# cliangyu/video-diffusion

Hardware: AMD Instinct MI355X
Metric: denoise-steps/sec (higher is better)
Workload: dtype f32

## Files before the change

### include/vd_amd.h

```cpp
#ifndef VD_AMD_H
#define VD_AMD_H
#ifdef __cplusplus
extern "C" {
#endif

typedef struct vd_config {
    int image_size;
    int num_channels;
    int num_res_blocks;
    int num_heads;
    int T;
    int n_attention_ds;
    int attention_ds[8];
    int use_scale_shift_norm;
    int use_spatial_encoding;
    int use_frame_encoding;
    int enforce_position_invariance;
    int use_rpe_net;
    int allow_interactions_between_padding;
    float rp_alpha, rp_beta, rp_gamma;
    int time_embed_mult;
    int cond_emb_type;
    int learn_sigma;
} vd_config;
// ... 71 lines not shown
                     double* mse_out, void* stream);
int vd_op_eps_mse(vd_engine* e, int B, int T, const float* x_start, const float* eps, const long long* t, int clip_denoised,
                  const float* latent_mask, unsigned long long seed, const unsigned long long* item_offset, const float* noise,
                  double* mse_out, void* stream);

int vd_window_begin(vd_engine* e, int B, int T, float* x, const float* obs_src, const float* obs_mask,
                    const float* latent_mask, const float* kinda_marg_mask, const long long* frame_indices,
                    int observed_frames, int sampler, int clip_denoised, float eta, unsigned long long seed,
                    unsigned long long offset, long long t_start, void* stream);
int vd_window_run(vd_engine* e, int n_steps, void* stream);
unsigned long long vd_window_generation(vd_engine* e);
int vd_window_graphs(vd_engine* e);

int vd_set_window_prefix_cache(vd_engine* e, int on);
int vd_window_prefix_frames(vd_engine* e);

int vd_set_window_suffix_skip(vd_engine* e, int on);
int vd_window_suffix_frames(vd_engine* e);

int vd_posterior_update(vd_engine* e, int mode, int B, long long per_sample, const float* x, const float* eps,
                        const long long* t, int clip_denoised, float eta, const float* noise,
                        unsigned long long seed, unsigned long long offset, float* sample, float* pred_xstart,
                        void* stream);

int vd_posterior_from_xstart(vd_engine* e, int mode, int B, long long per_sample, const float* x, const float* xstart_in,
                             const long long* t, int clip_denoised, float eta, const float* noise,
                             unsigned long long seed, unsigned long long offset, float* sample, float* pred_xstart,
                             float* mean, void* stream);

int vd_attn_blocks(vd_engine* e);
// ... 71 lines not shown
int vd_op_gn_bwd(const float* x0, const float* x1, int C0, int C, const float* affA, const float* affB, const float* mr,
                 const float* dy, int act, int nfr, int HW, const float* extra, float* dx0, int acc0, float* dx1, int acc1,
                 void* stream);
int vd_op_gn_temporal_bwd(const float* x, const float* gamma, const float* dy, int B, int T, int HW, int C, int accumulate,
                          float* dx, void* stream);
int vd_op_attn_temporal_bwd(const float* qkv, const float* Rk, const float* Rq, const float* Rv, const float* mask, int B,
                            int T, int HW, int C, int heads, int allow_pad, const float* dout, float* dqkv, void* stream);
int vd_op_attn_spatial_bwd(const float* qkv, int nfr, int L, int C, int heads, const float* dout, float* dqkv, void* stream);
int vd_op_out_conv_bwd(const float* deps, const float* w, int nfr, int H, int W, int C, int Cout, float* da, void* stream);
int vd_op_stem_col2im(const float* dcols, const float* obs, const float* lat, const float* km, int nfr, int H, int W,
                      int cond_mode, float* dx, void* stream);
int vd_op_sinus_embed(const float* t, int n, int dim, const float* freqs, float* out, void* stream);
int vd_op_frame_t(const long long* frame_indices, int B, int T, int center, float* tv, void* stream);
int vd_op_rpe_hidden(const float* te, int te_ld, const float* wbase, const long long* tab, const long long* frame_indices, int B, int T,
                     int C, float* E, int nz, long long zs_e, void* stream);
int vd_op_rpe_table(const float* table, const long long* frame_indices, int B, int T, int C, float alpha, float beta, float gamma,
                    float* R, void* stream);
int vd_op_posenc_add(const float* x, const float* P, const float* femb, int nfr, int HW, int C, float* y, void* stream);
int vd_op_assemble(const float* x, const float* obs_src, const float* obs_mask, const float* latent_mask, const float* kinda_marg_mask,
                   const float* t_model, int obs_t_mode, int B, int T, int H, int W, int Kpad, int cond_mode, const int* frame_list,
                   int n_list, int scalars_only, float* x_cols, float* t_frames, float* amask, void* stream);
int vd_op_move_rows(int scatter, const float* src, const int* list, int n, long long row_floats, float* dst, void* stream);
int vd_op_scatter_stats(const double* src, int split, int C, const int* list, int n, double* dst, void* stream);

typedef struct vd_lpips vd_lpips;
int vd_lpips_create(vd_lpips** out);
void vd_lpips_destroy(vd_lpips* h);
int vd_lpips_load_weight(vd_lpips* h, const char* name, const float* host, long long bytes);
long long vd_lpips_dim(int H, int W);
int vd_lpips_embed(vd_lpips* h, int N, int H, int W, const float* frames, float* out, void* stream);
// ... 28 lines not shown
```

### video-diffusion_amd/_lib.py

```python
import ctypes
import os
import subprocess

_HERE = os.path.dirname(os.path.abspath(__file__))
_CSRC = os.path.join(_HERE, "csrc")
SO_PATH = os.path.join(_HERE, "libvdamd.so")
SOURCES = ["igemm.hip", "conv_wino.hip", "conv_wino_r64.hip", "conv_wino_z128.hip", "gemm_frag.hip", "gemm_split.hip", "split_pack.hip", "norm.hip", "backward.hip", "attn_spatial.hip", "attn_temporal.hip", "attn_temporal_long.hip", "misc.hip", "engine.hip", "lpips.hip", "metrics.hip", "i3d.hip", "conv_cl.hip", "hallway.hip"]
HEADER = os.path.join(os.path.dirname(_HERE), "include", "vd_amd.h")
HEADERS = [os.path.join(_CSRC, "vd_common.h"), os.path.join(_CSRC, "wino_common.h"), os.path.join(_CSRC, "igemm_tile.h"), HEADER]
SOURCE_FLAGS = {"conv_wino_z128.hip": ["-mllvm", "-pragma-unroll-threshold=1000000"]}


def _toolchain():
    hipcc = os.environ.get("HIPCC", "/opt/rocm/bin/hipcc")
    flags = ["--offload-arch=gfx950", "-O3", "-std=c++17", "-fPIC", "-Wno-unused-value"] + \
        os.environ.get("VD_HIPCC_FLAGS", "").split()
    return hipcc, flags


def _sha(*parts):
    import hashlib
    h = hashlib.sha1()
    for p in parts:
        h.update(p if isinstance(p, bytes) else str(p).encode())
# ... 115 lines not shown
    "vd_pos_channels": (_I, [_P]),
    "vd_pos_resolution": (_I, [_P]),
    "vd_set_freqs": (_I, [_P, _P, _I, _P, _I]),
    "vd_set_schedule": (_I, [_P, _I, _P, _P, _F]),
    "vd_workspace_bytes": (_I, [_P, _I, _I, ctypes.POINTER(_L)]),
    "vd_unet_forward": (_I, [_P, _I, _I, _P, _P, _P, _P, _P, _P, _P, _I, _P, _P]),
    "vd_p_sample": (_I, [_P, _I, _I, _P, _P, _P, _P, _P, _P, _P, _I, _I, _P, _U, _U, _P, _P, _P, _P]),
    "vd_ddim_sample": (_I, [_P, _I, _I, _P, _P, _P, _P, _P, _P, _P, _I, _I, _F, _P, _U, _U, _P, _P, _P, _P]),
    "vd_p_mean_variance": (_I, [_P, _I, _I, _P, _P, _P, _P, _P, _P, _P, _I, _I, _P, _P, _P, _P]),
    "vd_vb_terms": (_I, [_P, _I, _I, _P, _P, _P, _P, _P, _I, _P, _P, _P, _P, _P, _P]),
    "vd_prior_bpd": (_I, [_P, _I, _I, _P, _P, _P, _P]),
    "vd_score_windows": (_I, [_P, _I, _I, _P, _P, _P, _P, _P, _P, _I, _U, _P, _P, _I, _P, _P]),
    "vd_op_eps_mse": (_I, [_P, _I, _I, _P, _P, _P, _I, _P, _U, _P, _P, _P, _P]),
    "vd_window_generation": (_U, [_P]),
    "vd_set_window_prefix_cache": (_I, [_P, _I]),
    "vd_window_prefix_frames": (_I, [_P]),
    "vd_set_window_suffix_skip": (_I, [_P, _I]),
    "vd_window_suffix_frames": (_I, [_P]),
    "vd_window_begin": (_I, [_P, _I, _I, _P, _P, _P, _P, _P, _P, _I, _I, _I, _F, _U, _U, _L, _P]),
    "vd_window_run": (_I, [_P, _I, _P]),
    "vd_window_graphs": (_I, [_P]),
    "vd_posterior_update": (_I, [_P, _I, _I, _L, _P, _P, _P, _I, _F, _P, _U, _U, _P, _P, _P]),
    "vd_posterior_from_xstart": (_I, [_P, _I, _I, _L, _P, _P, _P, _I, _F, _P, _U, _U, _P, _P, _P, _P]),
    "vd_attn_blocks": (_I, [_P]),
    "vd_attn_block_info": (_I, [_P, _I, ctypes.POINTER(_I), ctypes.POINTER(_I)]),
    "vd_set_attn_capture": (_I, [_P, _P, _P, _I]),
    "vd_bwd_weights_bytes": (_L, [_P]),
    "vd_set_bwd_weight_storage": (_I, [_P, _P, _L, _I]),
    "vd_load_weight_bwd": (_I, [_P, ctypes.c_char_p, _P, _L]),
    "vd_guided_step": (_I, [_P, _I, _I, _P, _P, _P, _P, _P, _P, _I, _P, _P, _P, _P, _P, _P, _P, _P]),
# ... 30 lines not shown
    "vd_op_affine_apply": (_I, [_P, _P, _P, _I, _I, _I, _P, _P]),
    "vd_op_affine_act": (_I, [_P, _P, _I, _I, _P, _P, _I, _I, _I, _P, _P]),
    "vd_op_gn_temporal": (_I, [_P, _P, _P, _I, _I, _I, _I, _P, _P]),
    "vd_op_attn_spatial": (_I, [_P, _I, _I, _I, _I, _P, _P]),
    "vd_op_attn_temporal": (_I, [_P, _P, _P, _P, _P, _I, _I, _I, _I, _I, _I, _P, _P]),
    "vd_op_out_conv": (_I, [_P, _P, _P, _P, _P, _I, _I, _I, _I, _I, _P, _P]),
    "vd_op_gn_bwd": (_I, [_P, _P, _I, _I, _P, _P, _P, _P, _I, _I, _I, _P, _P, _I, _P, _I, _P]),
    "vd_op_gn_temporal_bwd": (_I, [_P, _P, _P, _I, _I, _I, _I, _I, _P, _P]),
    "vd_op_attn_temporal_bwd": (_I, [_P, _P, _P, _P, _P, _I, _I, _I, _I, _I, _I, _P, _P, _P]),
    "vd_op_attn_spatial_bwd": (_I, [_P, _I, _I, _I, _I, _P, _P, _P]),
    "vd_op_out_conv_bwd": (_I, [_P, _P, _I, _I, _I, _I, _I, _P, _P]),
    "vd_op_stem_col2im": (_I, [_P, _P, _P, _P, _I, _I, _I, _I, _P, _P]),
    "vd_op_sinus_embed": (_I, [_P, _I, _I, _P, _P, _P]),
    "vd_op_frame_t": (_I, [_P, _I, _I, _I, _P, _P]),
    "vd_op_rpe_hidden": (_I, [_P, _I, _P, _P, _P, _I, _I, _I, _P, _I, _L, _P]),
    "vd_op_rpe_table": (_I, [_P, _P, _I, _I, _I, _F, _F, _F, _P, _P]),
    "vd_op_posenc_add": (_I, [_P, _P, _P, _I, _I, _I, _P, _P]),
    "vd_op_assemble": (_I, [_P, _P, _P, _P, _P, _P, _I, _I, _I, _I, _I, _I, _I, _P, _I, _I, _P, _P, _P, _P]),
    "vd_op_move_rows": (_I, [_I, _P, _P, _I, _L, _P, _P]),
    "vd_op_scatter_stats": (_I, [_P, _I, _I, _P, _I, _P, _P]),
    "vd_lpips_create": (_I, [ctypes.POINTER(_P)]),
    "vd_lpips_destroy": (None, [_P]),
    "vd_lpips_load_weight": (_I, [_P, ctypes.c_char_p, _P, _L]),
    "vd_lpips_dim": (_L, [_I, _I]),
    "vd_lpips_embed": (_I, [_P, _I, _I, _I, _P, _P, _P]),
    "vd_fps_select": (_I, [_I, _I, _L, _P, _I, _P, _I, _P, _P, _P]),
    "vd_frame_metrics": (_I, [_I, _I, _I, _I, _P, _P, _I, _D, _P, _P, _P]),
    "vd_pair_sqdist": (_I, [_I, _L, _P, _P, _P, _P]),
    "vd_i3d_create": (_I, [ctypes.POINTER(_P)]),
    "vd_i3d_destroy": (None, [_P]),
# ... 55 lines not shown
```

### video-diffusion_amd/csrc/engine.hip

```cpp
#include <cmath>
#include <cstring>
#include <unordered_map>
#include <vector>

#include "../../include/vd_amd.h"
#include "vd_common.h"

namespace vd {

thread_local std::string g_last_error;
void set_error(const std::string& msg) { g_last_error = msg; }

int launch_frame_t(const int64_t* fidx, int B, int T, int center, float* tv, hipStream_t s);

enum ParamKind { PK_RAW = 0, PK_CONV3, PK_STEM, PK_POSENC, PK_OUTCONV, PK_LINF, PK_CONV3W, PK_CONV3S,
                 PK_CONV3WU };

struct Param {
    std::string name;
    int nd = 0;
    long long shape[4] = {1, 1, 1, 1};
    size_t numel = 0;
    size_t packed = 0;
    size_t off = 0;
// ... 176 lines not shown
    int suf_blk = -2, suf_layer = -1;
    int p_posenc = -1, p_te0w, p_te0b, p_te2w, p_te2b, p_outgw, p_outgb, p_outw, p_outb;
    size_t film_w_off = 0, film_b_off = 0, te_w_off = 0, te_b_off = 0;
    int film_total = 0, te_total = 0;
    size_t packed_total = 0;
    float* wbuf = nullptr;
    bool wbuf_on_host = false;
    int put(void* dst, const void* src, size_t bytes) {
        if (wbuf_on_host) { std::memcpy(dst, src, bytes); return 0; }
        VD_HIP(hipMemcpy(dst, src, bytes, hipMemcpyHostToDevice));
        return 0;
    }
    struct RpeGroup { int C; std::vector<int> blocks; long long* d_hid = nullptr; long long* d_out = nullptr; };
    std::vector<RpeGroup> rpe_groups;
    std::vector<float*> rpe_R;
    int rpe_all(const float* te, const int64_t* fidx, int B, int T, hipStream_t st, Arena& ar);
    int rpe_tables();
    void rpe_group_blocks();
    float* d_freq_time = nullptr; int n_freq_time = 0;
    float* d_freq_frame = nullptr; int n_freq_frame = 0;
    float* d_tab = nullptr; int num_timesteps = 0;
    float* d_tmap = nullptr; float rescale = 1.f;
    char* ws = nullptr; size_t ws_cap = 0;
    bool ws_suf = false;
    int ws_B = 0, ws_T = 0; size_t ws_tail = 0;
    std::unordered_map<long long, size_t> ws_peaks;
    static size_t tm_bytes(int B) { return ((size_t)B * sizeof(float) + 255) & ~(size_t)255; }
    size_t step_tail_bytes(int B, int T) const { return tm_bytes(B) + (size_t)B * T * (cfg.learn_sigma ? 6 : 3) * cfg.image_size * cfg.image_size * sizeof(float); }
    float* step_tm() const { return reinterpret_cast<float*>(ws + ws_tail); }
    float* step_eps(int B) const { return reinterpret_cast<float*>(ws + ws_tail + tm_bytes(B)); }
    Arena step_arena() const { Arena a; a.base = ws; a.cap = ws_tail; return a; }
// ... 632 lines not shown
            const RpeP* rp[3] = {&a.rq, &a.rk, &a.rv};
            for (int k = 0; k < 3; ++k) {
                const int z = 3 * (int)i + k;
                th[3 * z] = rp[k]->te_off; th[3 * z + 1] = (long long)params[rp[k]->dw].off; th[3 * z + 2] = (long long)params[rp[k]->db].off;
                to[2 * z] = (long long)params[rp[k]->ow].off; to[2 * z + 1] = (long long)params[rp[k]->ob].off;
            }
        }
        VD_HIP(hipMalloc(reinterpret_cast<void**>(&g.d_hid), th.size() * sizeof(long long)));
        VD_HIP(hipMalloc(reinterpret_cast<void**>(&g.d_out), to.size() * sizeof(long long)));
        VD_HIP(hipMemcpy(g.d_hid, th.data(), th.size() * sizeof(long long), hipMemcpyHostToDevice));
        VD_HIP(hipMemcpy(g.d_out, to.data(), to.size() * sizeof(long long), hipMemcpyHostToDevice));
    }
    return 0;
}

int vd_engine::rpe_all(const float* te, const int64_t* fidx, int B, int T, hipStream_t st, Arena& ar) {
    rpe_R.clear();
    if (!cfg.use_rpe_net || attn.empty() || !te_total) return 0;
    rpe_group_blocks();
    const size_t rrows = (size_t)B * T * T;
    rpe_R.assign(3 * attn.size(), nullptr);
    int rc = 0;
    for (auto& g : rpe_groups) {
        const int nn = 3 * (int)g.blocks.size(), C = g.C;
        float* Rg = ar.get<float>((size_t)nn * rrows * C);
        for (size_t i = 0; i < g.blocks.size(); ++i)
            for (int k = 0; k < 3; ++k) rpe_R[3 * g.blocks[i] + k] = Rg + (3 * i + k) * rrows * C;
        const size_t mk = ar.mark();
        float* Eh = ar.get<float>((size_t)nn * rrows * C);
        ar.release(mk);
        if (ar.dry) continue;
        VD_REQUIRE(g.d_hid && g.d_out, "rpe_all: offset tables missing (ensure_ws builds them)");
        if ((rc = launch_rpe_hidden_tab(te, te_total, wbuf, g.d_hid, fidx, B, T, C, Eh, nn, rrows * C, st))) return rc;
        IgemmArgs q = linear_args((int)rrows, C, C);
        q.src0 = Eh; q.out = Rg;
        q.wfrag = wbuf + params[attn[g.blocks[0]].rq.ow].off; q.bias = wbuf + params[attn[g.blocks[0]].rq.ob].off;
        q.zcount = nn; q.zs_a = q.zs_out = (int)(rrows * C); q.ztab = g.d_out; q.zbase = wbuf;
        if ((rc = igemm_p(q, st))) return rc;
    }
    return 0;
}

int vd_engine::forward(const FwdIn& in, hipStream_t st, Arena& ar, const PrefixPlan* pp, const SuffixPlan* sp) {
    const int B = in.B, T = in.T, N = B * T, S = cfg.image_size, mc = cfg.num_channels;
    int rc;
    VD_REQUIRE(!pp || (!tape && !ar.dry && pp->store && n_before_attn > 0), "prefix plan: executor steps only");
    VD_REQUIRE(!sp || (!tape && sp->n > 0 && sp->n <= N && (ar.dry || sp->list)), "suffix plan: executor steps only, at least one frame");
    struct SelGuard { ~SelGuard() { g_sel_nfr = 0; } } sel_guard;
    const int Npre = pp ? pp->n : N;
    float* x8 = ar.get<float>((size_t)Npre * S * S * STEM_KPAD);
    float* tfr = ar.get<float>(N);
    float* amask = ar.get<float>(N);
    float* tsin = ar.get<float>((size_t)N * mc);
// ... 12 lines not shown
            aa.frame_list = pp->list; aa.n_list = pp->n;
        }
        if ((rc = launch_assemble(aa, st))) return rc;
        if ((rc = launch_sinus_embed(tfr, N, mc, d_freq_time, tsin, st))) return rc;
        if ((rc = linear(tsin, N, mc, E, W(p_te0w), W(p_te0b), 0, nullptr, e1, st))) return rc;
        if ((rc = linear(e1, N, E, E, W(p_te2w), W(p_te2b), 1, nullptr, emb, st))) return rc;
        if ((rc = linear(emb, N, E, film_total, wbuf + film_w_off, wbuf + film_b_off, 1, nullptr, film, st))) return rc;
        if (te_total && (rc = linear(emb, N, E, te_total, wbuf + te_w_off, wbuf + te_b_off, 0, nullptr, te, st))) return rc;
        if (cfg.use_frame_encoding) {
            VD_REQUIRE(d_freq_frame && n_freq_frame == pos_ch / 2, "vd_set_freqs not called (frame frequencies)");
            if ((rc = launch_frame_t(in.fidx, B, T, cfg.enforce_position_invariance, ftv, st))) return rc;
            if ((rc = launch_sinus_embed(ftv, N, pos_ch, d_freq_frame, femb, st))) return rc;
        }
    }
    rpe_R.clear();
    if (!(pp && pp->build_only) && (rc = rpe_all(te, in.fidx, B, T, st, ar))) return rc;
    attn_seq = 0;
    std::vector<Tens> hs;
    Tens h{x8, STEM_KPAD, S};
    int Nrun = Npre;
    const float* film_full = film;
    if (pp || ar.dry) {
        float* fc = ar.get<float>((size_t)std::max(pp ? Npre : N, 1) * film_total);
        if (pp) {
            if ((rc = launch_gather_rows(film_full, pp->list, Npre, film_total, fc, st))) return rc;
            film = fc;
        }
    }
    auto run = [&](const std::vector<Layer>& blk, Tens in0, const Tens* in1, Tens* outp, size_t l0 = 0, size_t l1 = ~(size_t)0) -> int {
        const int N = Nrun;
        Tens cur = in0;
// ... 930 lines not shown
    vd_engine::WinKey key;
    std::memset(&key, 0, sizeof(key));
    key.B = B; key.T = T; key.obs_mode = obs_mode; key.sampler = sampler; key.clip = clip; key.eta = eta;
    key.x = x; key.obs_src = obs_src; key.obs = obs; key.lat = lat; key.km = km; key.fidx = fidx;
    e->win_cur = -1;
    e->win_lost = false;
    ++e->win_gen;
    e->win_left = t_start + 1;
    const int N = B * T;
    const bool use_pre = e->prefix_cache_on && obs_mode == 0 && e->cfg.cond_emb_type == 0 && e->n_before_attn > 0;
    const bool want_suf = e->suffix_skip_on && obs_mode != 1 && e->cfg.cond_emb_type == 0 && e->suf_blk >= -1 && !e->attn.empty();
    std::vector<unsigned char> inv;
    int n_inv = 0;
    if ((use_pre || want_suf) && (rc = invariant_frames(obs, lat, N, st, &inv, &n_inv))) return rc;
    const bool pre_on = use_pre && n_inv > 0, suf_on = want_suf && n_inv > 0 && n_inv < N;
    key.flags = (pre_on ? 1 : 0) | (suf_on ? 2 : 0);
    const int hit = find_window_graph(e, key, inv);
    if (hit >= 0) {
        e->win_cur = hit;
        return pre_on ? prefix_build_pass(e, key, e->win_graphs[hit], st) : 0;
    }
    const float* net_obs_src = obs_mode == 2 ? e->d_win_xtm1 : obs_src;
    const int net_mode = obs_mode == 3 ? 2 : obs_mode;
    if ((rc = warmup_forward(e, key, net_obs_src, net_mode, st))) return rc;
    return capture_window(e, key, inv, n_inv, net_obs_src, net_mode, st);
}

int vd_set_window_prefix_cache(vd_engine* e, int on) {
    VD_REQUIRE(e, "null engine");
    e->prefix_cache_on = on != 0;
    return 0;
}

int vd_window_prefix_frames(vd_engine* e) {
    VD_REQUIRE(e, "null engine");
    return e->win_cur >= 0 && e->win_graphs[e->win_cur].store ? e->win_graphs[e->win_cur].n_inv : 0;
}

int vd_set_window_suffix_skip(vd_engine* e, int on) {
    VD_REQUIRE(e, "null engine");
    e->suffix_skip_on = on != 0;
    return 0;
}

int vd_window_suffix_frames(vd_engine* e) {
// ... 434 lines not shown

int vd_op_sinus_embed(const float* t, int n, int dim, const float* freqs, float* out, void* stream) {
    VD_REQUIRE(t && freqs && out && n > 0 && dim >= 2, "vd_op_sinus_embed: n rows of dim >= 2 columns, dim / 2 frequencies");
    return launch_sinus_embed(t, n, dim, freqs, out, static_cast<hipStream_t>(stream));
}

int vd_op_frame_t(const long long* fidx, int B, int T, int center, float* tv, void* stream) {
    VD_REQUIRE(fidx && tv && B > 0 && T > 0, "vd_op_frame_t: shape");
    return launch_frame_t(reinterpret_cast<const int64_t*>(fidx), B, T, center, tv, static_cast<hipStream_t>(stream));
}

int vd_op_rpe_hidden(const float* te, int te_ld, const float* wbase, const long long* tab, const long long* fidx, int B, int T, int C,
                     float* E, int nz, long long zs_e, void* stream) {
    VD_REQUIRE(te && wbase && tab && fidx && E && B > 0 && T > 0 && C > 0 && nz > 0, "vd_op_rpe_hidden: shape");
    VD_REQUIRE(te_ld >= C && zs_e >= (long long)B * T * T * C, "vd_op_rpe_hidden: te rows of at least C floats, a net's output inside its stride");
    return launch_rpe_hidden_tab(te, te_ld, wbase, tab, reinterpret_cast<const int64_t*>(fidx), B, T, C, E, nz, (size_t)zs_e,
                                 static_cast<hipStream_t>(stream));
}

int vd_op_rpe_table(const float* table, const long long* fidx, int B, int T, int C, float alpha, float beta, float gamma, float* R,
                    void* stream) {
    VD_REQUIRE(table && fidx && R && B > 0 && T > 0 && C > 0, "vd_op_rpe_table: shape");
    VD_REQUIRE(alpha >= 1.f && beta >= alpha && gamma >= alpha, "vd_op_rpe_table: bucket parameters 1 <= alpha <= beta, alpha <= gamma");
    return launch_rpe_table(table, reinterpret_cast<const int64_t*>(fidx), B, T, C, alpha, beta, gamma, R, static_cast<hipStream_t>(stream));
}

int vd_op_posenc_add(const float* x, const float* P, const float* femb, int nfr, int HW, int C, float* y, void* stream) {
    VD_REQUIRE(x && y && nfr > 0 && HW > 0 && C > 0 && C % 4 == 0, "vd_op_posenc_add: channels in 16-byte units");
    return launch_posenc_add(x, P, femb, nfr, HW, C, y, static_cast<hipStream_t>(stream));
}

int vd_op_assemble(const float* x, const float* obs_src, const float* obs_mask, const float* latent_mask, const float* kinda_marg_mask,
// ... 24 lines not shown
```

### video-diffusion_amd/csrc/gemm_frag.hip

```cpp
#include "vd_common.h"

namespace vd {

constexpr int GLD = 36;

#ifdef VD_GEMM_TIMING
__device__ unsigned long long g_gemm_stamp[6];
#define GEMM_STAMP(i) do { if (threadIdx.x == 0 && blockIdx.x == gridDim.x / 2 && blockIdx.y == 0) {                  \
        g_gemm_stamp[i] = __builtin_readcyclecounter();                                                             \
        if (i == 0) g_gemm_stamp[4] = __builtin_amdgcn_s_memrealtime();                                             \
        if (i == 3) g_gemm_stamp[5] = __builtin_amdgcn_s_memrealtime(); } } while (0)
extern "C" int vd_debug_gemm_stamps(unsigned long long* host_out) {
    return (int)hipMemcpyFromSymbol(host_out, HIP_SYMBOL(g_gemm_stamp), sizeof(g_gemm_stamp));
}
#else
#define GEMM_STAMP(i)
#endif

template <int BM, int BN, bool ACT>
__global__ __launch_bounds__(256, 3) void gemm_frag_kernel(IgemmArgs a) {
    constexpr int MI = BM / 64, NI = BN / 64, AR = BM / 32;
    extern __shared__ __attribute__((aligned(16))) float smem[];
    const int tid = threadIdx.x, lane = tid & 63, wave = __builtin_amdgcn_readfirstlane(tid >> 6);
    const int wm = wave >> 1, wn = wave & 1;
    const int lr = lane & 31, lh = lane >> 5;
    const int m0 = blockIdx.x * BM, n0 = blockIdx.y * BN;
    const int lrow = tid >> 3, lq = tid & 7;
    const int nchunk = a.Cin >> 5, ncoblk = a.Cout >> 5;
    const int C1 = a.Cin - a.C0;
    GEMM_STAMP(0);
    if (a.zcount > 1) {
        const int z = blockIdx.z;
        a.src0 += (size_t)z * a.zs_a; a.out += (size_t)z * a.zs_out;
        a.wfrag = a.zbase + a.ztab[2 * z];
        a.bias = a.zbase + a.ztab[2 * z + 1];
    }

    const auto asrc0 = __builtin_amdgcn_make_buffer_rsrc(const_cast<float*>(a.src0), 0, a.M * a.C0 * 4, 0x00020000);
    const auto asrc1 = __builtin_amdgcn_make_buffer_rsrc(const_cast<float*>(a.src1 ? a.src1 : a.src0), 0,
                                                         a.src1 ? a.M * C1 * 4 : 0, 0x00020000);
    unsigned ao0[AR], ao1[AR];
#pragma unroll
    for (int j = 0; j < AR; ++j) {
        const unsigned row = (unsigned)min(m0 + lrow + 32 * j, a.M - 1);
        ao0[j] = row * (unsigned)(a.C0 * 4) + lq * 16u;
        ao1[j] = row * (unsigned)(C1 * 4) + lq * 16u;
    }
    const auto bsrc = __builtin_amdgcn_make_buffer_rsrc(const_cast<float*>(a.wfrag), 0, a.Cin * a.Cout * 4, 0x00020000);
    unsigned bo[NI];
#pragma unroll
    for (int j = 0; j < NI; ++j) bo[j] = (unsigned)min((int)blockIdx.y * (BN / 32) + wn * NI + j, ncoblk - 1) * 4096u + lane * 16u;

    f32x4 ra[AR], bfr[4][NI], afr[2][MI];
    auto a_prefetch = [&](int chunk) {
        const int c = chunk * 32;
        if (c < a.C0) {
#pragma unroll
            for (int j = 0; j < AR; ++j)
                ra[j] = __builtin_bit_cast(f32x4, __builtin_amdgcn_raw_buffer_load_b128(asrc0, ao0[j], c * 4, 0));
        } else {
#pragma unroll
            for (int j = 0; j < AR; ++j)
                ra[j] = __builtin_bit_cast(f32x4, __builtin_amdgcn_raw_buffer_load_b128(asrc1, ao1[j], (c - a.C0) * 4, 0));
        }
    };
    auto a_store = [&](float* Ad) {
// ... 140 lines not shown
```

### video-diffusion_amd/csrc/gemm_split.hip

```cpp
#include <cstring>
#include <vector>

#include "vd_common.h"

namespace vd {

typedef __bf16 bf16x4 __attribute__((ext_vector_type(4)));
typedef __bf16 bf16x8 __attribute__((ext_vector_type(8)));
typedef unsigned u32x4 __attribute__((ext_vector_type(4)));
typedef unsigned u32x2 __attribute__((ext_vector_type(2)));

template <bool F16>
__device__ __forceinline__ f32x16 mfma_piece(u32x4 a, u32x4 b, f32x16 c) {
    if constexpr (F16) return __builtin_amdgcn_mfma_f32_32x32x16_f16(__builtin_bit_cast(f16x8, a), __builtin_bit_cast(f16x8, b), c, 0, 0, 0);
    else return __builtin_amdgcn_mfma_f32_32x32x16_bf16(__builtin_bit_cast(bf16x8, a), __builtin_bit_cast(bf16x8, b), c, 0, 0, 0);
}

#ifndef VD_GS_SKIP
#define VD_GS_SKIP 0
#endif
#ifdef VD_GS_TIMING
__device__ unsigned long long g_gs_stamp[8];
#define GS_STAMP(i) do { if (threadIdx.x == 0 && blockIdx.x == gridDim.x / 2 && blockIdx.y == 0) {                        \
        __builtin_amdgcn_sched_barrier(0); g_gs_stamp[i] = __builtin_amdgcn_s_memrealtime(); __builtin_amdgcn_sched_barrier(0); } } while (0)
// ... 22 lines not shown

template <int BM, int BN, bool ACT, bool CONV, bool F16 = true, bool SIDE = false>
__global__ __launch_bounds__(256, 2) void gemm_split_kernel(IgemmArgs a) {
    constexpr int MI = BM / 64, NI = BN / 64, AR = BM / 32;
    constexpr bool B2R = F16;
    constexpr int RING = NI >= 3 ? 2 : (BM == 64 && BN == 64) ? 6 : 3;
    constexpr int BP = B2R ? 2 : 3;
    constexpr int PF = BM == 64 ? 3 : 1;
    constexpr int NPL = F16 ? 2 : 3;
    constexpr int PLANE = BM * SROW, ABUF = NPL * PLANE;
    extern __shared__ __attribute__((aligned(16))) char smem_c[];
    const int tid = threadIdx.x, lane = tid & 63, wave = __builtin_amdgcn_readfirstlane(tid >> 6);
    GS_STAMP(0);
    const int wm = wave >> 1, wn = wave & 1;
    const int lr = lane & 31, lh = lane >> 5;
    int bxi = blockIdx.x, byi = blockIdx.y;
    if (gridDim.y > 1 && (gridDim.x & 7) == 0 && gridDim.x >= 128) {
        const unsigned lin = blockIdx.x + gridDim.x * blockIdx.y, xcd = lin & 7, loc = lin >> 3;
        byi = loc % gridDim.y;
        bxi = (loc / gridDim.y) * 8 + xcd;
    }
    const int m0 = bxi * BM, n0 = byi * BN;
    const int lgrp = tid >> 3, lrow = ((lgrp >> 1) & 3) + 8 * (lgrp >> 3) + 4 * (lgrp & 1), lq = tid & 7;
    const int cpt = a.Cin >> 5;
    const int nchunk = CONV ? 9 * cpt : cpt, ncoblk = a.Cout >> 5;
    const int C1 = a.Cin - a.C0;
    if (a.zcount > 1) {
        const int z = blockIdx.z;
        a.src0 += (size_t)z * a.zs_a; a.out += (size_t)z * a.zs_out;
        a.wfrag = a.zbase + a.ztab[2 * z];
        a.bias = a.zbase + a.ztab[2 * z + 1];
    }

    const auto asrc0 = __builtin_amdgcn_make_buffer_rsrc(const_cast<float*>(a.src0), 0,
                                                         (CONV ? a.nfr * a.Hs * a.Ws : a.M) * a.C0 * 4, 0x00020000);
    const auto asrc1 = __builtin_amdgcn_make_buffer_rsrc(const_cast<float*>(a.src1 ? a.src1 : a.src0), 0,
                                                         a.src1 ? a.M * C1 * 4 : 0, 0x00020000);
    unsigned ao0[AR], ao1[AR];
    int iy0[AR], ix0[AR];
#pragma unroll
    for (int j = 0; j < AR; ++j) {
        const unsigned row = (unsigned)min(m0 + lrow + 32 * j, a.M - 1);
        if constexpr (CONV) {
// ... 371 lines not shown
```

### video-diffusion_amd/csrc/misc.hip

```cpp
#include <algorithm>

#include "vd_common.h"

namespace vd {

__global__ __launch_bounds__(256) void assemble_kernel(AssembleArgs a) {
    const int n = a.frame_list ? a.frame_list[blockIdx.y] : blockIdx.y;
    const int HW = a.H * a.W;
    const float om = a.obs_mask[n], lm = a.lat_mask[n], km = a.km_mask[n];
    const float any = fminf(om + lm + km, 1.0f);
    const int Cs = a.cond_mode == 0 ? 5 : (a.cond_mode == 1 ? 6 : 3);
    if (blockIdx.x == 0 && threadIdx.x == 0 && !a.frame_list) {
        const float t = a.t_model[n / a.T];
        const float tobs = a.obs_t_mode == 0 ? 0.f : (a.obs_t_mode == 1 ? t : t - 1.f);
        float tf = t;
        if (a.cond_mode == 0) tf = tobs * om + t * (1.f - om);
        else if (a.cond_mode == 2) {
            bool any_obs = false;
            for (int k = 0; k < a.T; ++k) any_obs |= a.obs_mask[(n / a.T) * a.T + k] == 1.f;
            if (any_obs) tf = -1.f;
        }
        a.t_frames[n] = tf;
        a.amask[n] = any;
    }
// ... 118 lines not shown
        float s = 0.f;
        for (int t = 0; t < T; ++t) s += (float)fidx[b * T + t];
        mean = s / (float)T;
    }
    for (int t = threadIdx.x; t < T; t += blockDim.x) tv[b * T + t] = (float)fidx[b * T + t] - mean;
}

int launch_frame_t(const int64_t* fidx, int B, int T, int center, float* tv, hipStream_t s) {
    hipLaunchKernelGGL(frame_t_kernel, dim3(B), dim3(64), 0, s, fidx, T, center, tv);
    VD_HIP(hipGetLastError());
    return 0;
}

__global__ __launch_bounds__(256) void rpe_hidden_tab_kernel(const float* __restrict__ te, int te_ld, const float* __restrict__ wbase,
                                                             const long long* __restrict__ tab, const int64_t* __restrict__ fidx, int T, int C,
                                                             float* __restrict__ E, size_t zs_e) {
    __shared__ float feat[64][3];
    const long long* tz = tab + 3 * blockIdx.y;
    te += tz[0];
    const float* Wd = wbase + tz[1];
    const float* bd = wbase + tz[2];
    E += blockIdx.y * zs_e;
    const int bt = blockIdx.x, b = bt / T;
    for (int s0 = 0; s0 < T; s0 += 64) {
        const int ns = min(64, T - s0);
        __syncthreads();
        if ((int)threadIdx.x < ns) {
            const float d = (float)(fidx[bt] - fidx[b * T + s0 + threadIdx.x]);
            feat[threadIdx.x][0] = logf(1.0f + fmaxf(d, 0.f));
            feat[threadIdx.x][1] = logf(1.0f + fmaxf(-d, 0.f));
            feat[threadIdx.x][2] = d == 0.f ? 1.f : 0.f;
        }
        __syncthreads();
        for (int c = threadIdx.x; c < C; c += 256) {
            const float bc = bd[c], w0 = Wd[c * 3], w1 = Wd[c * 3 + 1], w2 = Wd[c * 3 + 2], tv = te[(size_t)bt * te_ld + c];
            for (int k = 0; k < ns; ++k) {
                const float lin = bc + feat[k][0] * w0 + feat[k][1] * w1 + feat[k][2] * w2;
                E[((size_t)bt * T + s0 + k) * C + c] = silu_f(tv + lin);
            }
        }
    }
}

int launch_rpe_hidden_tab(const float* te, int te_ld, const float* wbase, const long long* tab, const int64_t* fidx, int B, int T, int C,
                          float* E, int nz, size_t zs_e, hipStream_t s) {
    hipLaunchKernelGGL(rpe_hidden_tab_kernel, dim3(B * T, nz), dim3(256), 0, s, te, te_ld, wbase, tab, fidx, T, C, E, zs_e);
    VD_HIP(hipGetLastError());
    return 0;
}

__global__ __launch_bounds__(256) void rpe_table_kernel(const float* __restrict__ table, const int64_t* __restrict__ fidx,
                                                        int T, int C, float alpha, float beta, float gamma, double lg,
                                                        float* __restrict__ R) {
    const int row = blockIdx.x;
    const int s_ = row % T, bt = row / T, b = bt / T;
    const long long d = fidx[bt] - fidx[b * T + s_];
    long long id = d;
    const float ad = fabsf((float)d);
    if (ad > alpha) {
        double v = (double)alpha + log((double)ad / (double)alpha) / lg * ((double)beta - (double)alpha);
        const double r = rint(v);
// ... 562 lines not shown
```

### video-diffusion_amd/csrc/vd_common.h

```cpp
#pragma once
#include <hip/hip_runtime.h>
#include <cstdint>
#include <cstdio>
#include <string>

typedef float f32x4 __attribute__((ext_vector_type(4)));
typedef float f32x16 __attribute__((ext_vector_type(16)));

namespace vd {

constexpr int kMaxWindowFrames = 128;
constexpr int kMaxGuidedWindowFrames = 32;

void set_error(const std::string& msg);
extern thread_local std::string g_last_error;

#define VD_HIP(call)                                                                   \
    do {                                                                               \
        hipError_t e_ = (call);                                                        \
        if (e_ != hipSuccess) {                                                        \
            vd::set_error(std::string(#call) + ": " + hipGetErrorString(e_));          \
            return -2;                                                                 \
        }                                                                              \
    } while (0)
// ... 62 lines not shown
    const float* affA;
    const float* affB;
    int act;
    const float* res;
    int res_ld;
    const float* fbias;
    int fbias_ld;
    float* out;
    int ldo;
    int Cout, M;
    double* stats;
    int stats_split;
    int stats_hw;
    int zcount, zs_a, zs_out;
    const long long* ztab = nullptr; const float* zbase = nullptr;
    int wsplit;
    float* ksplit_ws;
    size_t ksplit_ws_floats;
};

struct AttnSpatialArgs {
    const float* qkv;
    float* out;
    int nfr, L, C, heads;
    float scale;
};

struct AttnTemporalArgs {
    const float* qkv;
    const float* Rk;
// ... 147 lines not shown
    int B, T, H, W, Kpad;
    int cond_mode;
    float* x_cols;
    float* t_frames;
    float* amask;
    const int* frame_list = nullptr;
    int n_list = 0;
    int scalars_only = 0;
};
int launch_assemble(const AssembleArgs& a, hipStream_t s);
int launch_gather_rows(const float* src, const int* list, int n, size_t row_floats, float* dst, hipStream_t s);
int launch_scatter_rows(const float* src, const int* list, int n, size_t row_floats, float* dst, hipStream_t s);
int launch_scatter_stats(const double* src, int split, int C, const int* list, int n, double* dst, hipStream_t s);
int launch_sinus_embed(const float* t, int n, int dim, const float* freqs, float* out, hipStream_t s);
int launch_rpe_hidden_tab(const float* te, int te_ld, const float* wbase, const long long* tab, const int64_t* fidx, int B, int T, int C,
                          float* E, int nz, size_t zs_e, hipStream_t s);
int launch_rpe_table(const float* table, const int64_t* fidx, int B, int T, int C, float alpha, float beta,
                     float gamma, float* R, hipStream_t s);
int launch_posenc_add(const float* x, const float* P, const float* femb, int nfr, int HW, int C, float* y,
                      hipStream_t s);
int launch_frame_t(const int64_t* fidx, int B, int T, int center, float* tv, hipStream_t s);
int launch_out_conv(const float* x, const float* affA, const float* affB, const float* w, const float* bias, int nfr,
                    int H, int W, int C, int Cout, float* out_nchw, hipStream_t s);

bool head_gemm_supported(int HW, int C, int ldt);
int launch_head_gemm(const float* h, const float* affA, const float* affB, const float* Wt, int nfr, int HW, int C, int ldt, float* T, hipStream_t s);
int launch_out_gather(const float* T, const float* bias, int nfr, int H, int W, int ldt, int Cout, float* out_nchw, hipStream_t s);

struct PosteriorArgs {
    const float* x;
    const float* eps;
// ... 109 lines not shown
```

### video-diffusion_amd/unet.py

```python
import ctypes
import math
from collections import OrderedDict

import numpy as np
import torch as th

from . import _lib

_OBS_MODES = {"x_0": 0, "x_t": 1, "x_t_minus_1": 2}


class CondMargVideoModel:
    def __init__(self, *, T, image_size, model_channels, num_res_blocks, attention_resolutions, num_heads=1,
                 use_scale_shift_norm=False, use_spatial_encoding=False, use_frame_encoding=False,
                 cross_frame_attention=True, enforce_position_invariance=False, use_rpe_net=False,
                 bucket_params=None, cond_emb_type="channel", allow_interactions_between_padding=False,
                 in_channels=3, out_channels=3, dropout=0, num_classes=None, num_heads_upsample=-1,
                 use_checkpoint=False, temporal_augment_type=None, channel_mult=None, **unused):
        cond = cond_emb_type.replace("-initzero", "")
        if cond == "channel":
            cond_mode = 0
        elif "duplicate" in cond_emb_type or "all" in cond_emb_type:
            cond_mode = 1
        elif cond_emb_type == "t=0":
# ... 212 lines not shown
            raise RuntimeError("weights already live on " + str(self._wbuf.device))
        if self._wbuf is None:
            nbytes = _lib.lib().vd_weights_bytes(self._handle)
            self._wbuf = th.zeros(nbytes // 4, dtype=th.float32)
            _lib.check(_lib.lib().vd_set_weight_storage_host(self._handle, _lib.ptr(self._wbuf), nbytes))
        if self._host_sd is not None:
            self._upload()
        return self._wbuf

    def mark_weights_received(self):
        _lib.check(_lib.lib().vd_mark_weights_loaded(self._handle))

    def weights_layout_id(self):
        return int(_lib.lib().vd_weights_layout_id(self._handle))

    def check_device_errors(self):
        flags = ctypes.c_int(0)
        _lib.check(_lib.lib().vd_device_errors(self._handle, ctypes.byref(flags)))
        if flags.value & 1:
            raise IndexError("timestep index out of range for the diffusion schedule (device flag set by an earlier step)")
        if flags.value & 2:
            raise FloatingPointError(
                "a denoise step consumed a network output that is not finite (device flag set by an earlier step; the affected "
                "elements of its result are NaN).  In the default arithmetic VD_MATH=f16x3 fp32 operands travel as two fp16 pieces: "
                "an operand beyond the split's range (|x| >= 2^15; inputs of a 3x3 conv: 2^13) overflows -- set VD_MATH=bf16x6 (exact three-piece split, full "
                "fp32 exponent range) on every rank and reload the weights")

    def _pack_kwargs(self, x, kw):
        B, T = x.shape[:2]
        dev = x.device
# ... 61 lines not shown
```

Before: 51.24.

## Deduplicate RPE-net work across batch items with identical frame timings and indices

Adds a device kernel that finds batch items sharing identical frame-time and frame-index vectors, assigns each a representative and rank, and counts the distinct rows. The RPE hidden kernel and the grouped GEMM then compute only the distinct items, early-exiting surplus blocks via a device-side live-row count, and an expand kernel copies results to the duplicate slots. This aims to cut redundant relative-position-network compute when batch items share positions, at the cost of an extra serial detection kernel, a copy pass and remapped block indexing in two GEMM kernels. The feature is on by default and is folded into the window graph cache key.

Measured after the change: 51.42 (median of 6 runs). No clear change (+0.4%).

```diff
diff --git a/include/vd_amd.h b/include/vd_amd.h
--- a/include/vd_amd.h
+++ b/include/vd_amd.h
@@ -109,6 +109,8 @@
 
 int vd_set_window_prefix_cache(vd_engine* e, int on);
 int vd_window_prefix_frames(vd_engine* e);
+
+int vd_set_rpe_dedupe(vd_engine* e, int on);
 
 int vd_set_window_suffix_skip(vd_engine* e, int on);
 int vd_window_suffix_frames(vd_engine* e);
@@ -210,6 +212,7 @@
 int vd_op_frame_t(const long long* frame_indices, int B, int T, int center, float* tv, void* stream);
 int vd_op_rpe_hidden(const float* te, int te_ld, const float* wbase, const long long* tab, const long long* frame_indices, int B, int T,
                      int C, float* E, int nz, long long zs_e, void* stream);
+int vd_op_rpe_rep(const float* t_frames, const long long* frame_indices, int B, int T, int* rep, int* rank, int* m_live, void* stream);
 int vd_op_rpe_table(const float* table, const long long* frame_indices, int B, int T, int C, float alpha, float beta, float gamma,
                     float* R, void* stream);
 int vd_op_posenc_add(const float* x, const float* P, const float* femb, int nfr, int HW, int C, float* y, void* stream);
diff --git a/video-diffusion_amd/_lib.py b/video-diffusion_amd/_lib.py
--- a/video-diffusion_amd/_lib.py
+++ b/video-diffusion_amd/_lib.py
@@ -153,6 +153,7 @@
     "vd_op_eps_mse": (_I, [_P, _I, _I, _P, _P, _P, _I, _P, _U, _P, _P, _P, _P]),
     "vd_window_generation": (_U, [_P]),
     "vd_set_window_prefix_cache": (_I, [_P, _I]),
+    "vd_set_rpe_dedupe": (_I, [_P, _I]),
     "vd_window_prefix_frames": (_I, [_P]),
     "vd_set_window_suffix_skip": (_I, [_P, _I]),
     "vd_window_suffix_frames": (_I, [_P]),
@@ -213,6 +214,7 @@
     "vd_op_sinus_embed": (_I, [_P, _I, _I, _P, _P, _P]),
     "vd_op_frame_t": (_I, [_P, _I, _I, _I, _P, _P]),
     "vd_op_rpe_hidden": (_I, [_P, _I, _P, _P, _P, _I, _I, _I, _P, _I, _L, _P]),
+    "vd_op_rpe_rep": (_I, [_P, _P, _I, _I, _P, _P, _P, _P]),
     "vd_op_rpe_table": (_I, [_P, _P, _I, _I, _I, _F, _F, _F, _P, _P]),
     "vd_op_posenc_add": (_I, [_P, _P, _P, _I, _I, _I, _P, _P]),
     "vd_op_assemble": (_I, [_P, _P, _P, _P, _P, _P, _I, _I, _I, _I, _I, _I, _I, _P, _I, _I, _P, _P, _P, _P]),
diff --git a/video-diffusion_amd/csrc/engine.hip b/video-diffusion_amd/csrc/engine.hip
--- a/video-diffusion_amd/csrc/engine.hip
+++ b/video-diffusion_amd/csrc/engine.hip
@@ -214,7 +214,8 @@
     struct RpeGroup { int C; std::vector<int> blocks; long long* d_hid = nullptr; long long* d_out = nullptr; };
     std::vector<RpeGroup> rpe_groups;
     std::vector<float*> rpe_R;
-    int rpe_all(const float* te, const int64_t* fidx, int B, int T, hipStream_t st, Arena& ar);
+    int rpe_all(const float* te, const float* tfr, const int64_t* fidx, int B, int T, hipStream_t st, Arena& ar);
+    bool rpe_dedupe = true;
     int rpe_tables();
     void rpe_group_blocks();
     float* d_freq_time = nullptr; int n_freq_time = 0;
@@ -877,13 +878,19 @@
     return 0;
 }
 
-int vd_engine::rpe_all(const float* te, const int64_t* fidx, int B, int T, hipStream_t st, Arena& ar) {
+int vd_engine::rpe_all(const float* te, const float* tfr, const int64_t* fidx, int B, int T, hipStream_t st, Arena& ar) {
     rpe_R.clear();
     if (!cfg.use_rpe_net || attn.empty() || !te_total) return 0;
     rpe_group_blocks();
     const size_t rrows = (size_t)B * T * T;
     rpe_R.assign(3 * attn.size(), nullptr);
     int rc = 0;
+    int *rep = nullptr, *rank = nullptr, *m_live = nullptr;
+    if (B > 1) {
+        int* keys = ar.get<int>(2 * (size_t)B + 1);
+        if (rpe_dedupe) { rep = keys; rank = keys + B; m_live = keys + 2 * B; }
+        if (rep && !ar.dry && (rc = launch_rpe_rep(tfr, fidx, B, T, rep, rank, m_live, st))) return rc;
+    }
     for (auto& g : rpe_groups) {
         const int nn = 3 * (int)g.blocks.size(), C = g.C;
         float* Rg = ar.get<float>((size_t)nn * rrows * C);
@@ -894,12 +901,14 @@
         ar.release(mk);
         if (ar.dry) continue;
         VD_REQUIRE(g.d_hid && g.d_out, "rpe_all: offset tables missing (ensure_ws builds them)");
-        if ((rc = launch_rpe_hidden_tab(te, te_total, wbuf, g.d_hid, fidx, B, T, C, Eh, nn, rrows * C, st))) return rc;
+        if ((rc = launch_rpe_hidden_tab(te, te_total, wbuf, g.d_hid, fidx, B, T, C, Eh, nn, rrows * C, rep, rank, m_live, st))) return rc;
         IgemmArgs q = linear_args((int)rrows, C, C);
         q.src0 = Eh; q.out = Rg;
         q.wfrag = wbuf + params[attn[g.blocks[0]].rq.ow].off; q.bias = wbuf + params[attn[g.blocks[0]].rq.ob].off;
         q.zcount = nn; q.zs_a = q.zs_out = (int)(rrows * C); q.ztab = g.d_out; q.zbase = wbuf;
+        q.m_live = m_live;
         if ((rc = igemm_p(q, st))) return rc;
+        if (rep && (rc = launch_rpe_expand(Rg, B, T, C, nn, rrows * C, rep, rank, st))) return rc;
     }
     return 0;
 }
@@ -942,7 +951,7 @@
         }
     }
     rpe_R.clear();
-    if (!(pp && pp->build_only) && (rc = rpe_all(te, in.fidx, B, T, st, ar))) return rc;
+    if (!(pp && pp->build_only) && (rc = rpe_all(te, tfr, in.fidx, B, T, st, ar))) return rc;
     attn_seq = 0;
     std::vector<Tens> hs;
     Tens h{x8, STEM_KPAD, S};
@@ -1903,7 +1912,7 @@
     int n_inv = 0;
     if ((use_pre || want_suf) && (rc = invariant_frames(obs, lat, N, st, &inv, &n_inv))) return rc;
     const bool pre_on = use_pre && n_inv > 0, suf_on = want_suf && n_inv > 0 && n_inv < N;
-    key.flags = (pre_on ? 1 : 0) | (suf_on ? 2 : 0);
+    key.flags = (pre_on ? 1 : 0) | (suf_on ? 2 : 0) | (e->rpe_dedupe ? 4 : 0);
     const int hit = find_window_graph(e, key, inv);
     if (hit >= 0) {
         e->win_cur = hit;
@@ -1918,6 +1927,13 @@
 int vd_set_window_prefix_cache(vd_engine* e, int on) {
     VD_REQUIRE(e, "null engine");
     e->prefix_cache_on = on != 0;
+    return 0;
+}
+
+int vd_set_rpe_dedupe(vd_engine* e, int on) {
+    VD_REQUIRE(e, "null engine");
+    VD_REQUIRE(e->win_cur < 0 || e->win_lost || e->win_left == 0, "vd_set_rpe_dedupe: a window is open (run its remaining steps or begin again afterwards)");
+    e->rpe_dedupe = on != 0;
     return 0;
 }
 
@@ -2382,8 +2398,13 @@
                      float* E, int nz, long long zs_e, void* stream) {
     VD_REQUIRE(te && wbase && tab && fidx && E && B > 0 && T > 0 && C > 0 && nz > 0, "vd_op_rpe_hidden: shape");
     VD_REQUIRE(te_ld >= C && zs_e >= (long long)B * T * T * C, "vd_op_rpe_hidden: te rows of at least C floats, a net's output inside its stride");
-    return launch_rpe_hidden_tab(te, te_ld, wbase, tab, reinterpret_cast<const int64_t*>(fidx), B, T, C, E, nz, (size_t)zs_e,
+    return launch_rpe_hidden_tab(te, te_ld, wbase, tab, reinterpret_cast<const int64_t*>(fidx), B, T, C, E, nz, (size_t)zs_e, nullptr, nullptr, nullptr,
                                  static_cast<hipStream_t>(stream));
+}
+
+int vd_op_rpe_rep(const float* tfr, const long long* fidx, int B, int T, int* rep, int* rank, int* m_live, void* stream) {
+    VD_REQUIRE(tfr && fidx && rep && rank && m_live && B > 0 && T > 0, "vd_op_rpe_rep: shape");
+    return launch_rpe_rep(tfr, reinterpret_cast<const int64_t*>(fidx), B, T, rep, rank, m_live, static_cast<hipStream_t>(stream));
 }
 
 int vd_op_rpe_table(const float* table, const long long* fidx, int B, int T, int C, float alpha, float beta, float gamma, float* R,
diff --git a/video-diffusion_amd/csrc/gemm_frag.hip b/video-diffusion_amd/csrc/gemm_frag.hip
--- a/video-diffusion_amd/csrc/gemm_frag.hip
+++ b/video-diffusion_amd/csrc/gemm_frag.hip
@@ -24,13 +24,23 @@
     const int tid = threadIdx.x, lane = tid & 63, wave = __builtin_amdgcn_readfirstlane(tid >> 6);
     const int wm = wave >> 1, wn = wave & 1;
     const int lr = lane & 31, lh = lane >> 5;
-    const int m0 = blockIdx.x * BM, n0 = blockIdx.y * BN;
+    int bxi = blockIdx.x, byi = blockIdx.y, bzi = blockIdx.z;
+    if (a.m_live) {
+        const unsigned per = (unsigned)((*a.m_live + BM - 1) / BM) * gridDim.y;
+        const unsigned g = blockIdx.x + gridDim.x * (blockIdx.y + gridDim.y * blockIdx.z);
+        if (g >= per * gridDim.z) return;
+        bzi = g / per;
+        const unsigned r = g - bzi * per;
+        bxi = r / gridDim.y;
+        byi = r - bxi * gridDim.y;
+    }
+    const int m0 = bxi * BM, n0 = byi * BN;
     const int lrow = tid >> 3, lq = tid & 7;
     const int nchunk = a.Cin >> 5, ncoblk = a.Cout >> 5;
     const int C1 = a.Cin - a.C0;
     GEMM_STAMP(0);
     if (a.zcount > 1) {
-        const int z = blockIdx.z;
+        const int z = bzi;
         a.src0 += (size_t)z * a.zs_a; a.out += (size_t)z * a.zs_out;
         a.wfrag = a.zbase + a.ztab[2 * z];
         a.bias = a.zbase + a.ztab[2 * z + 1];
@@ -49,7 +59,7 @@
     const auto bsrc = __builtin_amdgcn_make_buffer_rsrc(const_cast<float*>(a.wfrag), 0, a.Cin * a.Cout * 4, 0x00020000);
     unsigned bo[NI];
 #pragma unroll
-    for (int j = 0; j < NI; ++j) bo[j] = (unsigned)min((int)blockIdx.y * (BN / 32) + wn * NI + j, ncoblk - 1) * 4096u + lane * 16u;
+    for (int j = 0; j < NI; ++j) bo[j] = (unsigned)min(byi * (BN / 32) + wn * NI + j, ncoblk - 1) * 4096u + lane * 16u;
 
     f32x4 ra[AR], bfr[4][NI], afr[2][MI];
     auto a_prefetch = [&](int chunk) {
diff --git a/video-diffusion_amd/csrc/gemm_split.hip b/video-diffusion_amd/csrc/gemm_split.hip
--- a/video-diffusion_amd/csrc/gemm_split.hip
+++ b/video-diffusion_amd/csrc/gemm_split.hip
@@ -60,8 +60,16 @@
     GS_STAMP(0);
     const int wm = wave >> 1, wn = wave & 1;
     const int lr = lane & 31, lh = lane >> 5;
-    int bxi = blockIdx.x, byi = blockIdx.y;
-    if (gridDim.y > 1 && (gridDim.x & 7) == 0 && gridDim.x >= 128) {
+    int bxi = blockIdx.x, byi = blockIdx.y, bzi = blockIdx.z;
+    if (a.m_live) {
+        const unsigned per = (unsigned)((*a.m_live + BM - 1) / BM) * gridDim.y;
+        const unsigned g = blockIdx.x + gridDim.x * (blockIdx.y + gridDim.y * blockIdx.z);
+        if (g >= per * gridDim.z) return;
+        bzi = g / per;
+        const unsigned r = g - bzi * per;
+        bxi = r / gridDim.y;
+        byi = r - bxi * gridDim.y;
+    } else if (gridDim.y > 1 && (gridDim.x & 7) == 0 && gridDim.x >= 128) {
         const unsigned lin = blockIdx.x + gridDim.x * blockIdx.y, xcd = lin & 7, loc = lin >> 3;
         byi = loc % gridDim.y;
         bxi = (loc / gridDim.y) * 8 + xcd;
@@ -72,7 +80,7 @@
     const int nchunk = CONV ? 9 * cpt : cpt, ncoblk = a.Cout >> 5;
     const int C1 = a.Cin - a.C0;
     if (a.zcount > 1) {
-        const int z = blockIdx.z;
+        const int z = bzi;
         a.src0 += (size_t)z * a.zs_a; a.out += (size_t)z * a.zs_out;
         a.wfrag = a.zbase + a.ztab[2 * z];
         a.bias = a.zbase + a.ztab[2 * z + 1];
diff --git a/video-diffusion_amd/csrc/misc.hip b/video-diffusion_amd/csrc/misc.hip
--- a/video-diffusion_amd/csrc/misc.hip
+++ b/video-diffusion_amd/csrc/misc.hip
@@ -156,14 +156,28 @@
 
 __global__ __launch_bounds__(256) void rpe_hidden_tab_kernel(const float* __restrict__ te, int te_ld, const float* __restrict__ wbase,
                                                              const long long* __restrict__ tab, const int64_t* __restrict__ fidx, int T, int C,
-                                                             float* __restrict__ E, size_t zs_e) {
+                                                             float* __restrict__ E, size_t zs_e, const int* __restrict__ rep,
+                                                             const int* __restrict__ rank, const int* __restrict__ m_live) {
     __shared__ float feat[64][3];
-    const long long* tz = tab + 3 * blockIdx.y;
+    int bt = blockIdx.x, net = blockIdx.y;
+    int ot = bt;
+    if (rep) {
+        const int per = *m_live / T, B = gridDim.x / T;
+        const int g = blockIdx.x + gridDim.x * blockIdx.y;
+        if (g >= per * (int)gridDim.y) return;
+        net = g / per;
+        ot = g - net * per;
+        const int slot = ot / T;
+        int b = slot;
+        while (b + 1 < B && !(rep[b] == b && rank[b] == slot)) ++b;
+        bt = b * T + (ot - slot * T);
+    }
+    const int b = bt / T;
+    const long long* tz = tab + 3 * net;
     te += tz[0];
     const float* Wd = wbase + tz[1];
     const float* bd = wbase + tz[2];
-    E += blockIdx.y * zs_e;
-    const int bt = blockIdx.x, b = bt / T;
+    E += net * zs_e;
     for (int s0 = 0; s0 < T; s0 += 64) {
         const int ns = min(64, T - s0);
         __syncthreads();
@@ -178,15 +192,65 @@
             const float bc = bd[c], w0 = Wd[c * 3], w1 = Wd[c * 3 + 1], w2 = Wd[c * 3 + 2], tv = te[(size_t)bt * te_ld + c];
             for (int k = 0; k < ns; ++k) {
                 const float lin = bc + feat[k][0] * w0 + feat[k][1] * w1 + feat[k][2] * w2;
-                E[((size_t)bt * T + s0 + k) * C + c] = silu_f(tv + lin);
+                E[((size_t)ot * T + s0 + k) * C + c] = silu_f(tv + lin);
             }
         }
     }
 }
 
 int launch_rpe_hidden_tab(const float* te, int te_ld, const float* wbase, const long long* tab, const int64_t* fidx, int B, int T, int C,
-                          float* E, int nz, size_t zs_e, hipStream_t s) {
-    hipLaunchKernelGGL(rpe_hidden_tab_kernel, dim3(B * T, nz), dim3(256), 0, s, te, te_ld, wbase, tab, fidx, T, C, E, zs_e);
+                          float* E, int nz, size_t zs_e, const int* rep, const int* rank, const int* m_live, hipStream_t s) {
+    hipLaunchKernelGGL(rpe_hidden_tab_kernel, dim3(B * T, nz), dim3(256), 0, s, te, te_ld, wbase, tab, fidx, T, C, E, zs_e, rep, rank, m_live);
+    VD_HIP(hipGetLastError());
+    return 0;
+}
+
+__global__ __launch_bounds__(64) void rpe_rep_kernel(const float* __restrict__ tfr, const int64_t* __restrict__ fidx, int B, int T,
+                                                     int* __restrict__ rep, int* __restrict__ rank, int* __restrict__ m_live) {
+    const unsigned* tb = reinterpret_cast<const unsigned*>(tfr);
+    for (int b = threadIdx.x; b < B; b += blockDim.x) {
+        int r = b;
+        for (int o = 0; o < b; ++o) {
+            unsigned long long d = 0;
+#pragma unroll 4
+            for (int t = 0; t < T; ++t) d |= (unsigned long long)(tb[o * T + t] ^ tb[b * T + t]) | (unsigned long long)(fidx[o * T + t] ^ fidx[b * T + t]);
+            if (d == 0) { r = o; break; }
+        }
+        rep[b] = r;
+    }
+    __syncthreads();
+    for (int b = threadIdx.x; b <= B; b += blockDim.x) {
+        int n = 0;
+        for (int o = 0; o < b; ++o) n += rep[o] == o;
+        if (b < B) rank[b] = n;
+        else *m_live = n * T * T;
+    }
+}
+
+int launch_rpe_rep(const float* tfr, const int64_t* fidx, int B, int T, int* rep, int* rank, int* m_live, hipStream_t s) {
+    hipLaunchKernelGGL(rpe_rep_kernel, dim3(1), dim3(64), 0, s, tfr, fidx, B, T, rep, rank, m_live);
+    VD_HIP(hipGetLastError());
+    return 0;
+}
+
+__global__ __launch_bounds__(256) void rpe_expand_kernel(float* __restrict__ R, size_t n4, size_t zs_r, int B, const int* __restrict__ rep,
+                                                         const int* __restrict__ rank) {
+    const size_t p = (size_t)blockIdx.x * 256 + threadIdx.x;
+    if (p >= n4) return;
+    float4* Rz = reinterpret_cast<float4*>(R + blockIdx.y * zs_r) + p;
+    int have = -1;
+    float4 v = {0.f, 0.f, 0.f, 0.f};
+    for (int b = B - 1; b >= 0; --b) {
+        const int r = rank[rep[b]];
+        if (r == b) continue;
+        if (r != have) { v = Rz[r * n4]; have = r; }
+        Rz[b * n4] = v;
+    }
+}
+
+int launch_rpe_expand(float* R, int B, int T, int C, int nz, size_t zs_r, const int* rep, const int* rank, hipStream_t s) {
+    const size_t n4 = (size_t)T * T * C / 4;
+    hipLaunchKernelGGL(rpe_expand_kernel, dim3((unsigned)((n4 + 255) / 256), nz), dim3(256), 0, s, R, n4, zs_r, B, rep, rank);
     VD_HIP(hipGetLastError());
     return 0;
 }
diff --git a/video-diffusion_amd/csrc/vd_common.h b/video-diffusion_amd/csrc/vd_common.h
--- a/video-diffusion_amd/csrc/vd_common.h
+++ b/video-diffusion_amd/csrc/vd_common.h
@@ -100,6 +100,7 @@
     int stats_hw;
     int zcount, zs_a, zs_out;
     const long long* ztab = nullptr; const float* zbase = nullptr;
+    const int* m_live = nullptr;
     int wsplit;
     float* ksplit_ws;
     size_t ksplit_ws_floats;
@@ -277,7 +278,9 @@
 int launch_scatter_stats(const double* src, int split, int C, const int* list, int n, double* dst, hipStream_t s);
 int launch_sinus_embed(const float* t, int n, int dim, const float* freqs, float* out, hipStream_t s);
 int launch_rpe_hidden_tab(const float* te, int te_ld, const float* wbase, const long long* tab, const int64_t* fidx, int B, int T, int C,
-                          float* E, int nz, size_t zs_e, hipStream_t s);
+                          float* E, int nz, size_t zs_e, const int* rep, const int* rank, const int* m_live, hipStream_t s);
+int launch_rpe_rep(const float* tfr, const int64_t* fidx, int B, int T, int* rep, int* rank, int* m_live, hipStream_t s);
+int launch_rpe_expand(float* R, int B, int T, int C, int nz, size_t zs_r, const int* rep, const int* rank, hipStream_t s);
 int launch_rpe_table(const float* table, const int64_t* fidx, int B, int T, int C, float alpha, float beta,
                      float gamma, float* R, hipStream_t s);
 int launch_posenc_add(const float* x, const float* P, const float* femb, int nfr, int HW, int C, float* y,
diff --git a/video-diffusion_amd/unet.py b/video-diffusion_amd/unet.py
--- a/video-diffusion_amd/unet.py
+++ b/video-diffusion_amd/unet.py
@@ -250,6 +250,9 @@
     def weights_layout_id(self):
         return int(_lib.lib().vd_weights_layout_id(self._handle))
 
+    def set_rpe_dedupe(self, on):
+        _lib.check(_lib.lib().vd_set_rpe_dedupe(self._handle, 1 if on else 0))
+
     def check_device_errors(self):
         flags = ctypes.c_int(0)
         _lib.check(_lib.lib().vd_device_errors(self._handle, ctypes.byref(flags)))
```
